# CSB5/XNA_Basecaller

Measured on NVIDIA B200. Metric: signal samples/sec basecalled (sup@v3.3 XNA), higher is better.
Workload: dtype fp16

## Files before the change

### include/xna_basecaller.h

```cpp
#ifndef XNA_BASECALLER_H
#define XNA_BASECALLER_H

#include <stdint.h>

#ifdef __cplusplus
extern "C" {
#endif

#define XB_ABI_VERSION 2

typedef struct xb_handle xb_handle;

enum xb_status {
    XB_OK = 0,
    XB_ERR_ARG = -1,
    XB_ERR_CUDA = -2,
    XB_ERR_STATE = -3,
    XB_ERR_UNSUPPORTED = -4,
    XB_ERR_NOMEM = -5
};

enum xb_flags {
    XB_FLAG_BF16 = 1,
    XB_FLAG_NO_ENCODER = 2,
// ... 73 lines not shown
int xb_encoder_fwd_train(xb_handle *h, const void *signal, int sig_dtype, int N, int L, float *scores, void *stream);
int xb_encoder_bwd(xb_handle *h, const void *signal, int sig_dtype, const float *scores, const float *dscores,
                   float *const *grads, int n_tensors, void *stream);

int xb_adamw_step(float *const *params, float *const *grads, float *const *exp_avg, float *const *exp_avg_sq,
                  const int64_t *numel, int n_tensors, float lr, float beta1, float beta2, float eps, float weight_decay,
                  float max_norm, int64_t step, float *grad_norm, float *scratch, void *stream);

int xb_stitch(xb_handle *h, const int8_t *rows, int T, const int32_t *chunk_first,
              const int32_t *chunk_count, const int32_t *read_len, int n_reads, int chunksize,
              int overlap, int stride, int reverse, int8_t *out, int out_stride, int32_t *out_len, void *stream);

int xb_gather_chunks(xb_handle *h, const void *signal, int sig_dtype, const int64_t *read_offset,
                     const int32_t *read_len, const int32_t *chunk_read, const int32_t *chunk_start, int n_chunks,
                     int L, float *out, void *stream);

int xb_preprocess_reads(xb_handle *h, const int16_t *raw, const int64_t *read_offset, const int32_t *read_len,
                        const double *scaling, const int32_t *offset, int n_reads, float *out, int32_t *out_len,
                        float *stats, void *stream);

int xb_compute_scores_host(xb_handle *h, const float *signal_host, int N, int L, int8_t *seq_host,
                           int32_t *lens_host, void *stream);

int xb_compute_scores_submit(xb_handle *h, int slot, const float *signal_host, int N, int L, int8_t *seq_host,
                             int32_t *lens_host, void *stream);
int xb_compute_scores_wait(xb_handle *h, int slot);

int64_t xb_launch_count(const xb_handle *h);

#define XB_NUM_STAGES 13
int xb_set_profiling(xb_handle *h, int on);
int xb_stage_times(xb_handle *h, float *ms, int *spans);

int xb_gemm_selftest(xb_handle *h, const void *A, const void *B, float *D, int M, int N, int K,
                     void *stream);

#ifdef __cplusplus
}
#endif
#endif
```

### xna_basecaller_b200/_lib.py

```python
import ctypes
import os

import torch

_HERE = os.path.dirname(os.path.abspath(__file__))
LIB_PATH = os.path.join(_HERE, 'libxna_b200.so')

XB_FLAG_BF16 = 1
XB_FLAG_NO_ENCODER = 2
XB_FLAG_TRAIN = 8
XB_SIG_F32, XB_SIG_F16, XB_SIG_I16 = 0, 1, 2
NUM_WEIGHTS = 28

SYMBOLS = (
    'xb_abi_version', 'xb_last_error', 'xb_create', 'xb_destroy', 'xb_load_weights', 'xb_load_conv_weights',
    'xb_load_lstm_weights', 'xb_load_head_weights', 'xb_conv_stem_fwd',
    'xb_lstm_fwd', 'xb_lstm_stack_fwd', 'xb_crf_head_fwd', 'xb_encoder_fwd', 'xb_crf_logz',
    'xb_crf_forward_scores', 'xb_crf_backward_scores', 'xb_crf_posteriors', 'xb_crf_viterbi', 'xb_crf_decode',
    'xb_ctc_crf_loss_fwd', 'xb_ctc_crf_loss_bwd', 'xb_stitch', 'xb_gather_chunks', 'xb_preprocess_reads', 'xb_compute_scores_host', 'xb_compute_scores_submit', 'xb_compute_scores_wait', 'xb_launch_count', 'xb_gemm_selftest',
    'xb_set_profiling', 'xb_stage_times', 'xb_crf_head_fwd_exp', 'xb_crf_decode_exp', 'xb_basecall_chunks',
    'xb_crf_logz_s', 'xb_crf_forward_scores_s', 'xb_crf_backward_scores_s', 'xb_crf_posteriors_max',
    'xb_encoder_fwd_train', 'xb_encoder_bwd', 'xb_adamw_step', 'xb_crf_beam_search',
)
STAGES = ('conv12_im2col', 'conv3_gemm', 'lstm_inproj_gemm', 'lstm_recurrence', 'crf_head_gemm', 'crf_alpha',
          'crf_backward', 'crf_viterbi', 'train_bptt', 'train_transpose', 'train_weight_grad_gemm', 'train_input_grad_gemm', 'train_head_conv_bwd')

_lib = None


def load():
    global _lib
    if _lib is not None:
        return _lib
    if not os.path.exists(LIB_PATH):
        raise RuntimeError(
            'xna_basecaller_b200: %s is missing -- build it with `python -m xna_basecaller_b200.build` '
            '(there is no CPU or PyTorch fallback for this path)' % LIB_PATH)
    lib = ctypes.CDLL(LIB_PATH)
    vp, ci, cf = ctypes.c_void_p, ctypes.c_int, ctypes.c_float
    lib.xb_abi_version.restype = ci
    lib.xb_last_error.restype = ctypes.c_char_p
    lib.xb_last_error.argtypes = [vp]
    lib.xb_create.argtypes = [ctypes.POINTER(vp), ci, ci, ci, ci, ci, ctypes.c_char_p, ci]
    lib.xb_destroy.argtypes = [vp]
    lib.xb_load_weights.argtypes = [vp, ctypes.POINTER(vp), ci, cf, cf, ci, vp]
    lib.xb_load_conv_weights.argtypes = [vp, vp, vp, vp, vp, vp, vp, vp]
    lib.xb_load_lstm_weights.argtypes = [vp, ci, vp, vp, vp, vp, vp]
    lib.xb_load_head_weights.argtypes = [vp, vp, vp, cf, cf, ci, vp]
    lib.xb_conv_stem_fwd.argtypes = [vp, vp, ci, ci, ci, vp, vp]
    lib.xb_lstm_fwd.argtypes = [vp, ci, vp, vp, ci, ci, ci, vp]
    lib.xb_lstm_stack_fwd.argtypes = [vp, vp, vp, ci, ci, vp]
    lib.xb_crf_head_fwd.argtypes = [vp, vp, vp, ci, ci, vp]
    lib.xb_encoder_fwd.argtypes = [vp, vp, ci, ci, ci, vp, vp]
    lib.xb_crf_logz.argtypes = [vp, vp, ci, ci, vp, vp]
    lib.xb_crf_forward_scores.argtypes = [vp, vp, ci, ci, vp, vp]
    lib.xb_crf_backward_scores.argtypes = [vp, vp, ci, ci, vp, vp]
    lib.xb_crf_posteriors.argtypes = [vp, vp, ci, ci, vp, vp]
    lib.xb_encoder_fwd_train.argtypes = [vp, vp, ci, ci, ci, vp, vp]
    lib.xb_encoder_bwd.argtypes = [vp, vp, ci, vp, vp, ctypes.POINTER(vp), ci, vp]
    lib.xb_adamw_step.argtypes = [ctypes.POINTER(vp), ctypes.POINTER(vp), ctypes.POINTER(vp), ctypes.POINTER(vp),
                                  ctypes.POINTER(ctypes.c_int64), ci, cf, cf, cf, cf, cf, cf, ctypes.c_int64, vp, vp, vp]
    lib.xb_crf_beam_search.argtypes = [vp, vp, ci, ci, ci, cf, vp, vp, vp, vp, vp]
    lib.xb_crf_logz_s.argtypes = [vp, vp, ci, ci, ci, vp, vp]
    lib.xb_crf_forward_scores_s.argtypes = [vp, vp, ci, ci, ci, vp, vp]
    lib.xb_crf_backward_scores_s.argtypes = [vp, vp, ci, ci, ci, vp, vp]
    lib.xb_crf_posteriors_max.argtypes = [vp, vp, ci, ci, vp, vp, vp]
    lib.xb_crf_viterbi.argtypes = [vp, vp, ci, ci, vp, vp]
    lib.xb_crf_decode.argtypes = [vp, vp, ci, ci, vp, vp, vp, vp, vp, vp]
    lib.xb_crf_decode_exp.argtypes = [vp, vp, ci, ci, vp, vp, vp, vp, vp, vp]
    lib.xb_crf_head_fwd_exp.argtypes = [vp, vp, vp, ci, ci, vp]
    lib.xb_basecall_chunks.argtypes = [vp, vp, ci, ci, ci, vp, vp, vp, vp]
    lib.xb_ctc_crf_loss_fwd.argtypes = [vp, vp, ci, ci, vp, ci, vp, ci, vp, vp]
    lib.xb_compute_scores_submit.argtypes = [vp, ci, vp, ci, ci, vp, vp, vp]
    lib.xb_compute_scores_wait.argtypes = [vp, ci]
    lib.xb_preprocess_reads.argtypes = [vp, vp, vp, vp, vp, vp, ci, vp, vp, vp, vp]
    lib.xb_ctc_crf_loss_bwd.argtypes = [vp, vp, ci, ci, vp, ci, vp, ci, vp, vp, vp, vp]
    lib.xb_stitch.argtypes = [vp, vp, ci, vp, vp, vp, ci, ci, ci, ci, ci, vp, ci, vp, vp]
    lib.xb_gather_chunks.argtypes = [vp, vp, ci, vp, vp, vp, vp, ci, ci, vp, vp]
    lib.xb_compute_scores_host.argtypes = [vp, vp, ci, ci, vp, vp, vp]
    lib.xb_launch_count.restype = ctypes.c_int64
    lib.xb_launch_count.argtypes = [vp]
    lib.xb_gemm_selftest.argtypes = [vp, vp, vp, vp, ci, ci, ci, vp]
    lib.xb_set_profiling.argtypes = [vp, ci]
    lib.xb_stage_times.argtypes = [vp, vp, vp]
    for name in SYMBOLS:
        if name not in ('xb_last_error', 'xb_launch_count'):
            getattr(lib, name).restype = ci
    _lib = lib
    return lib


def _ptr(t):
    return None if t is None else ctypes.c_void_p(t.data_ptr())


def _stream(device):
    return ctypes.c_void_p(torch.cuda.current_stream(device).cuda_stream)


class Handle:

    def __init__(self, alphabet, state_len=3, max_N=64, max_T=800, device=0, bf16=False, encoder=True, train=False):
        if not torch.cuda.is_available():
            raise RuntimeError('xna_basecaller_b200 needs a CUDA device (sm_100a); there is no CPU fallback')
        self.lib = load()
        self.alphabet = ''.join(alphabet)
        self.n_base = len(self.alphabet) - 1
        self.state_len = state_len
        self.C = self.n_base ** state_len
        self.NZ = self.n_base + 1
        self.max_N, self.max_T = max_N, max_T
        self.device = torch.device('cuda', device) if not isinstance(device, torch.device) else device
        self.bf16 = bf16
        self.dtype16 = torch.float16
        flags = (XB_FLAG_BF16 if bf16 else 0) | (0 if encoder else XB_FLAG_NO_ENCODER) | (XB_FLAG_TRAIN if train else 0)
        self.train = train
        h = ctypes.c_void_p()
        rc = self.lib.xb_create(ctypes.byref(h), self.device.index or 0, max_N, max_T, self.n_base, state_len,
                                self.alphabet.encode(), flags)
        if rc != 0:
            raise RuntimeError('xb_create failed (%d): %s' % (rc, self.lib.xb_last_error(None).decode()))
        self.h = h
        self._keep = None

    def close(self):
        if getattr(self, 'h', None):
            self.lib.xb_destroy(self.h)
            self.h = None

    def __del__(self):
        try:
            self.close()
        except Exception:
            pass

    def _check(self, rc, what):
        if rc != 0:
            raise RuntimeError('%s failed (%d): %s' % (what, rc, self.lib.xb_last_error(self.h).decode()))

    @property
    def launches(self):
        return int(self.lib.xb_launch_count(self.h))

    def set_profiling(self, on):
        self._check(self.lib.xb_set_profiling(self.h, int(on)), 'xb_set_profiling')

    def stage_times(self):
        ms = (ctypes.c_float * len(STAGES))()
        n = (ctypes.c_int * len(STAGES))()
        self._check(self.lib.xb_stage_times(self.h, ms, n), 'xb_stage_times')
        return {name: (float(ms[i]), int(n[i])) for i, name in enumerate(STAGES)}

    def load_weights(self, state_dict, scale=5.0, blank_score=2.0, expand_blanks=True):
        keys = []
        for i in range(3):
            keys += ['encoder.%d.conv.weight' % i, 'encoder.%d.conv.bias' % i]
        for i in range(4, 9):
            keys += ['encoder.%d.rnn.%s' % (i, k) for k in ('weight_ih_l0', 'weight_hh_l0', 'bias_ih_l0', 'bias_hh_l0')]
        keys += ['encoder.9.linear.weight', 'encoder.9.linear.bias']
        tensors = [state_dict[k].detach().to(self.device, torch.float32).contiguous() for k in keys]
        arr = (ctypes.c_void_p * NUM_WEIGHTS)(*[t.data_ptr() for t in tensors])
        rc = self.lib.xb_load_weights(self.h, arr, NUM_WEIGHTS, float(scale),
                                      float(blank_score if blank_score is not None else 0.0),
                                      int(bool(expand_blanks) and blank_score is not None), _stream(self.device))
        self._check(rc, 'xb_load_weights')
        torch.cuda.current_stream(self.device).synchronize()

    def _f32(self, t):
        return t.detach().to(self.device, torch.float32).contiguous()

    def load_conv_weights(self, w1, b1, w2, b2, w3, b3):
        ts = [self._f32(t) for t in (w1, b1, w2, b2, w3, b3)]
        self._check(self.lib.xb_load_conv_weights(self.h, *[_ptr(t) for t in ts], _stream(self.device)),
                    'xb_load_conv_weights')
        torch.cuda.current_stream(self.device).synchronize()

    def load_lstm_weights(self, layer, w_ih, w_hh, b_ih, b_hh):
        ts = [self._f32(t) for t in (w_ih, w_hh, b_ih, b_hh)]
        self._check(self.lib.xb_load_lstm_weights(self.h, int(layer), *[_ptr(t) for t in ts], _stream(self.device)),
# ... 271 lines not shown
```

### xna_basecaller_b200/csrc/lstm_persistent.cu

```cuda
#include <stdlib.h>

#include "xb_common.cuh"
#include "xb_ptx.cuh"
#include "xb_gemm.cuh"

using namespace xbptx;

#ifndef XB_LSTM_MUFU_TANH
#define XB_LSTM_MUFU_TANH 1
#endif

namespace {

constexpr int TILES = 24;
constexpr int KCH = XB_FEATURES / 64;
constexpr int HP = 3;
constexpr int KPB = KCH / HP;
constexpr int D_COL = 384;
constexpr int CTR_STRIDE = 32;
constexpr int MAX_CTRS = 64;

template <int SUB, int NS, int EW, int GB = 2> struct Cfg {
    static constexpr int NB = SUB * NS;
    static constexpr int H_BLOCK_BYTES = NS * 64 * 2;
    static constexpr int H_PART_BYTES = KPB * H_BLOCK_BYTES;
    static constexpr int H_BYTES = KCH * H_BLOCK_BYTES;
    static constexpr int G_BYTES = NS * 128 * 2;
    static constexpr int NBAR = HP + 1 + 4;
    static constexpr int EPI_WARP0 = ((SUB + 1 + 3) / 4) * 4;
    static constexpr int THREADS = (EPI_WARP0 + EW * SUB) * 32;
    static constexpr int NC = NS * 4 / EW;
    static constexpr int STAGE_BYTES = NC * 16;
    static constexpr int SMEM_BYTES = SUB * (H_BYTES + GB * G_BYTES) + (GB == 2 ? SUB * EW * STAGE_BYTES : 0) + 1024  + 1024 ;
    static_assert(D_COL + SUB * NS <= 512, "tensor memory columns");
    static_assert(NS % 16 == 0 && NS <= 48, "MMA N");
    static_assert((EW == 4 || EW == 8 || EW == 12) && NC % 16 == 0, "epilogue split");
    static_assert(SUB * NBAR * 8 + 16 <= 1024, "barrier block");
    static_assert(H_BLOCK_BYTES % 1024 == 0, "swizzle atom alignment");
};

struct PLParams {
    int T, N, reverse;
    int batch0, nbatch, G;
    const uint16_t *w_hh;
    uint16_t *y;
    int *counters;
    int one_release;
    int prefetch_y;
    long long *dbg;
    int tma_store;
    uint16_t *save;
};

#ifdef XB_EXPERIMENTS
#define DBG(sub_, ev) do { if (p.dbg && blockIdx.x == 0 && s >= 64 && s < 72) p.dbg[((s - 64) * 8 + (sub_)) * 16 + (ev)] = clock64(); } while (0)
#else
#define DBG(sub_, ev) do { } while (0)
#endif

__device__ __forceinline__ float tanh_approx(float x) {
    float y;
    asm("tanh.approx.f32 %0, %1;" : "=f"(y) : "f"(x));
    return y;
}
#if !XB_LSTM_MUFU_TANH
__device__ __forceinline__ float ex2f(float x) {
    float y;
    asm("ex2.approx.ftz.f32 %0, %1;" : "=f"(y) : "f"(x));
    return y;
}
__device__ __forceinline__ float rcpf(float x) {
    float y;
    asm("rcp.approx.ftz.f32 %0, %1;" : "=f"(y) : "f"(x));
    return y;
}
__device__ __forceinline__ float clampf(float x, float lim) { return fminf(fmaxf(x, -lim), lim); }
#endif

template <int XN> __device__ __forceinline__ void tmem_ld_16x256b(uint32_t taddr, uint32_t (&r)[4 * XN]);
template <> __device__ __forceinline__ void tmem_ld_16x256b<2>(uint32_t taddr, uint32_t (&r)[8]) {
    asm volatile("tcgen05.ld.sync.aligned.16x256b.x2.b32 {%0, %1, %2, %3, %4, %5, %6, %7}, [%8];"
                 : "=r"(r[0]), "=r"(r[1]), "=r"(r[2]), "=r"(r[3]), "=r"(r[4]), "=r"(r[5]), "=r"(r[6]), "=r"(r[7])
                 : "r"(taddr) : "memory");
}
template <> __device__ __forceinline__ void tmem_ld_16x256b<4>(uint32_t taddr, uint32_t (&r)[16]) {
    asm volatile("tcgen05.ld.sync.aligned.16x256b.x4.b32 {%0, %1, %2, %3, %4, %5, %6, %7, %8, %9, %10, %11, %12, %13, %14, %15}, [%16];"
                 : "=r"(r[0]), "=r"(r[1]), "=r"(r[2]), "=r"(r[3]), "=r"(r[4]), "=r"(r[5]), "=r"(r[6]), "=r"(r[7]), "=r"(r[8]),
                   "=r"(r[9]), "=r"(r[10]), "=r"(r[11]), "=r"(r[12]), "=r"(r[13]), "=r"(r[14]), "=r"(r[15])
                 : "r"(taddr) : "memory");
}
template <bool BF16, int SUB, int NS, int EW, int GB, bool SAVE = false>
__global__ void __launch_bounds__(Cfg<SUB, NS, EW, GB>::THREADS, 1)
lstm_persistent_kernel(const __grid_constant__ CUtensorMap tmY, const __grid_constant__ CUtensorMap tmG,
                       const __grid_constant__ CUtensorMap tmS, const PLParams p) {
    using X = xb16<BF16>;
    using C = Cfg<SUB, NS, EW, GB>;
    extern __shared__ uint8_t smem_raw[];
    uint8_t *smem = reinterpret_cast<uint8_t *>((reinterpret_cast<uintptr_t>(smem_raw) + 1023) & ~uintptr_t(1023));
    uint8_t *hbuf = smem;
    uint8_t *gbuf = smem + SUB * C::H_BYTES;
    uint8_t *stage = gbuf + SUB * GB * C::G_BYTES;
    uint64_t *bars = reinterpret_cast<uint64_t *>(stage + (GB == 2 ? SUB * EW * C::STAGE_BYTES : 0));
    uint32_t *tmem_holder = reinterpret_cast<uint32_t *>(bars + SUB * C::NBAR);
    auto h_full = [&](int sub, int part) { return bars + sub * C::NBAR + part; };
    auto d_full = [&](int sub) { return bars + sub * C::NBAR + HP; };
    auto g_full = [&](int sub, int q) { return bars + sub * C::NBAR + HP + 1 + q; };
    auto g_empty = [&](int sub, int q) { return bars + sub * C::NBAR + HP + 3 + q; };

    const int warp = __shfl_sync(0xffffffffu, (int)(threadIdx.x >> 5), 0), lane = threadIdx.x & 31;
    const int g = blockIdx.x / TILES, j = blockIdx.x % TILES;
    const int T = p.T, N = p.N;
    const int units = (p.nbatch + NS - 1) / NS;
    const int b0 = p.batch0 + NS * (int)(((long long)g * units) / p.G);
    const int b1 = min(p.batch0 + p.nbatch, p.batch0 + NS * (int)(((long long)(g + 1) * units) / p.G));
    const int count = b1 - b0;
    auto sub_row0 = [&](int sub) { return b0 + sub * NS; };
    auto sub_cnt = [&](int sub) { return max(0, min(NS, count - sub * NS)); };

    if (warp == 0 && lane == 0) {
        prefetch_tmap(&tmY);
        prefetch_tmap(&tmG);
        for (int sub = 0; sub < SUB; sub++) {
            for (int part = 0; part < HP; part++) mbar_init(h_full(sub, part), 1);
            mbar_init(d_full(sub), 1);
            for (int q = 0; q < 2; q++) {
                mbar_init(g_full(sub, q), 1);
                mbar_init(g_empty(sub, q), EW);
            }
        }
        fence_barrier_init();
    }
    if (warp == SUB) {
        tmem_alloc(tmem_holder, 512);
        tmem_relinquish();
    }
    tc_fence_before();
    __syncthreads();
    tc_fence_after();
    const uint32_t tmem_base = *tmem_holder;

    if (warp >= C::EPI_WARP0 && warp < C::EPI_WARP0 + 4) {
        const int q = warp & 3, r = q * 32 + lane;
        const uint4 *src = reinterpret_cast<const uint4 *>(p.w_hh + ((size_t)j * 128 + r) * XB_FEATURES);
        const uint32_t taddr = tmem_base + ((uint32_t)(q * 32) << 16);
#pragma unroll 1
        for (int c0 = 0; c0 < XB_FEATURES / 2; c0 += 32) {
            uint32_t v[32];
#pragma unroll
            for (int i = 0; i < 8; i++) {
                uint4 t4 = __ldg(src + c0 / 4 + i);
                v[4 * i] = t4.x; v[4 * i + 1] = t4.y; v[4 * i + 2] = t4.z; v[4 * i + 3] = t4.w;
            }
            tmem_st_32x32b_x32(taddr + c0, v);
        }
        tmem_st_wait();
    }
    tc_fence_before();
    __syncthreads();
    tc_fence_after();

    if (warp < SUB) {
        if (elect_one()) {
            const int sub = warp;
            const int row0 = sub_row0(sub);
            const int cnt_sub = sub_cnt(sub);
            const int *ctr = p.counters + (g * SUB + sub) * CTR_STRIDE;
            uint8_t *hb = hbuf + sub * C::H_BYTES;
            constexpr uint32_t idesc = umma_idesc_f16(BF16 ? 1u : 0u, 128, NS);
            const uint64_t bdesc0 = umma_desc_sw128(smem_u32(hb));
            const uint32_t dcol = tmem_base + D_COL + sub * NS;
            if (cnt_sub > 0) {
                mbar_expect_tx(g_full(sub, 0), C::G_BYTES);
                tma_load_2d(gbuf + (sub * GB) * C::G_BYTES, &tmG, g_full(sub, 0), j * 128, (p.reverse ? T - 1 : 0) * N + row0);
            }
            for (int s = 0; s < (cnt_sub > 0 ? T : 0); s++) {
                const int t = p.reverse ? T - 1 - s : s;
                if (GB == 2 && s + 1 < T) {
                    const int sn = s + 1, q = sn & 1, u = sn >> 1;
                    const int tn = p.reverse ? T - 1 - sn : sn;
                    if (u >= 1) mbar_wait(g_empty(sub, q), (u - 1) & 1);
                    mbar_expect_tx(g_full(sub, q), C::G_BYTES);
                    tma_load_2d(gbuf + (sub * 2 + q) * C::G_BYTES, &tmG, g_full(sub, q), j * 128, tn * N + row0);
                }
                if (p.prefetch_y && s + p.prefetch_y < T) {
                    const int t2 = p.reverse ? T - 1 - (s + p.prefetch_y) : s + p.prefetch_y;
                    for (int r = j; r < cnt_sub; r += TILES)
                        prefetch_l2_bulk(p.y + ((size_t)t2 * N + row0 + r) * XB_FEATURES, XB_FEATURES * 2);
                }
                if (s > 0) {
                    const int tp = p.reverse ? t + 1 : t - 1;
                    const int need = TILES * EW * s;
                    DBG(sub, 0);
                    while (ld_relaxed_gpu(ctr) < need) {
                    }
                    (void)ld_acquire_gpu(ctr);
                    DBG(sub, 1);
                    fence_proxy_async_global();
#pragma unroll
                    for (int part = 0; part < HP; part++) {
                        mbar_expect_tx(h_full(sub, part), C::H_PART_BYTES);
                        tma_load_3d(hb + part * C::H_PART_BYTES, &tmY, h_full(sub, part), 0, tp * N + row0, part * KPB);
                    }
                    DBG(sub, 2);
#pragma unroll
                    for (int part = 0; part < HP; part++) {
                        mbar_wait(h_full(sub, part), (s - 1) & 1);
                        tc_fence_after();
                        if (part == 0) DBG(sub, 8);
                        if (part == 0) DBG(sub, 3);
#pragma unroll
                        for (int kk = 0; kk < KPB * 4; kk++) {
                            const int kc = kk >> 2, k = kk & 3;
                            mma_f16_ts(dcol, tmem_base + part * (KPB * 32) + kk * 8,
                                       bdesc0 + (uint64_t)((part * C::H_PART_BYTES + kc * C::H_BLOCK_BYTES + k * 32) >> 4), idesc,
                                       (part | kk) != 0);
                        }
                    }
                    mma_commit(d_full(sub));
                    DBG(sub, 4);
                }
                if (GB == 1 && s + 1 < T) {
                    const int tn = p.reverse ? T - 2 - s : s + 1;
                    mbar_wait(g_empty(sub, 0), s & 1);
                    mbar_expect_tx(g_full(sub, 0), C::G_BYTES);
                    tma_load_2d(gbuf + sub * C::G_BYTES, &tmG, g_full(sub, 0), j * 128, tn * N + row0);
                }
            }
        }
    } else if (warp >= C::EPI_WARP0) {
        constexpr int NC = C::NC, CELLS = NC / 4;
        const int ew = (warp - C::EPI_WARP0) % EW, sub = (warp - C::EPI_WARP0) / EW, q = warp & 3;
        const int col0 = (ew >> 2) * NC;
        const int gt = lane & 3, ul = lane >> 2;
        const int unit = q * 8 + ul;
        const int row0 = sub_row0(sub);
        const int cnt = sub_cnt(sub);
#ifdef XB_EXPERIMENTS
        const bool tma_store = !SAVE && GB == 2 && cnt == NS && p.tma_store;
#else
        constexpr bool tma_store = false;
#endif
        const uint32_t taddr = tmem_base + ((uint32_t)(q * 32) << 16) + D_COL + sub * NS + col0;
        int *ctr = p.counters + (g * SUB + sub) * CTR_STRIDE;
        float cst[CELLS];
#pragma unroll
        for (int i = 0; i < CELLS; i++) cst[i] = 0.0f;

        for (int s = 0; s < (cnt > 0 ? T : 0); s++) {
            const int t = p.reverse ? T - 1 - s : s;
            const uint16_t *Gs = reinterpret_cast<const uint16_t *>(gbuf + (sub * GB + (GB == 2 ? (s & 1) : 0)) * C::G_BYTES);
            mbar_wait(g_full(sub, GB == 2 ? (s & 1) : 0), GB == 2 ? ((s >> 1) & 1) : (s & 1));
// ... 113 lines not shown
                if (ew == 0 && lane == 0) {
                    red_release_gpu_add(ctr, EW);
                    DBG(sub, 13);
                }
                if (lane == 0) mbar_arrive(g_empty(sub, GB == 2 ? (s & 1) : 0));
            } else {
                __syncwarp();
                if (lane == 0) {
                    red_release_gpu_add(ctr, 1);
                    mbar_arrive(g_empty(sub, GB == 2 ? (s & 1) : 0));
                    if (ew == 0) DBG(sub, 13);
                }
            }
            if (SAVE) {
                static_assert(!SAVE || GB == 2, "the saved-state stores reuse the staging rows after the gate buffer has been released");
#pragma unroll
                for (int qn = 0; qn < 5; qn++) {
                    __syncwarp();
#pragma unroll
                    for (int i = 0; i < CELLS; i++) {
                        const __half hv = __float2half_rn(sv[SAVE ? qn : 0][i]);
                        sts_u16(st_s + 2u * ((8 * (i >> 1) + 2 * gt + (i & 1)) * ST_PITCH + ul), *reinterpret_cast<const uint16_t *>(&hv));
                    }
                    __syncwarp();
                    if (lane < NC && col0 + lane < cnt)
                        *reinterpret_cast<uint4 *>(p.save + (((size_t)t * N + row0 + col0 + lane) * 5 + qn) * XB_FEATURES + j * 32 + q * 8) =
                            lds_v4(st_s + 2u * (lane * ST_PITCH));
                }
            }
        }
    }
    tc_fence_before();
    __syncthreads();
    if (warp == SUB) {
        tc_fence_after();
        tmem_dealloc(tmem_base, 512);
    }
}

template <bool BF16, int SUB, int NS, int EW, int GB = 2, bool SAVE = false>
int launch_cfg(xb_handle *h, int layer, void *y_tnc, int T, int N, int reverse, cudaStream_t s, void *save = nullptr) {
    using C = Cfg<SUB, NS, EW, GB>;
    CUtensorMap tmY, tmG, tmS;
    if (int rc = xb_make_tmap_hview(h, &tmY, y_tnc, (uint64_t)T * N, NS, KPB)) return rc;
    if (int rc = xb_make_tmap_2d_box(h, &tmS, y_tnc, (uint64_t)T * N, XB_FEATURES, XB_FEATURES, 32, NS, 0)) return rc;
    if (int rc = xb_make_tmap_2d_box(h, &tmG, h->gates, (uint64_t)T * N, XB_GATES, XB_GATES, 128, NS, 0)) return rc;
    const int max_groups = h->num_sms / TILES;
    if (max_groups < 1)
        return xb_fail(h, XB_ERR_UNSUPPORTED, "the persistent LSTM needs %d co-resident CTAs, the device has %d SMs", TILES, h->num_sms);
    const int block_cap = max_groups * C::NB;
    auto fn = lstm_persistent_kernel<BF16, SUB, NS, EW, GB, SAVE>;
    static bool configured[64] = {};
    if (!configured[h->device & 63]) {
        XB_CUDA(h, cudaFuncSetAttribute(fn, cudaFuncAttributeMaxDynamicSharedMemorySize, C::SMEM_BYTES));
        configured[h->device & 63] = true;
    }
    for (int batch0 = 0; batch0 < N; batch0 += block_cap) {
        PLParams p;
        p.T = T; p.N = N; p.reverse = reverse;
        p.batch0 = batch0;
        p.nbatch = (N - batch0 < block_cap) ? N - batch0 : block_cap;
        p.G = (p.nbatch + C::NB - 1) / C::NB;
        p.w_hh = reinterpret_cast<const uint16_t *>(h->lstm[layer].w_hh);
        p.y = reinterpret_cast<uint16_t *>(y_tnc);
        p.counters = h->lstm_counters;
        p.one_release = 1;
        p.prefetch_y = 4;
        p.dbg = nullptr;
        p.save = reinterpret_cast<uint16_t *>(save);
        p.tma_store = 0;
#ifdef XB_EXPERIMENTS
        if (getenv("XB_TMAS")) p.tma_store = atoi(getenv("XB_TMAS"));
#endif
#ifdef XB_EXPERIMENTS
        if (getenv("XB_LSTM_WARP_RELEASE")) p.one_release = 0;
        if (getenv("XB_LSTM_PREFETCH_Y")) p.prefetch_y = atoi(getenv("XB_LSTM_PREFETCH_Y"));
        if (getenv("XB_LSTM_DEBUG")) p.dbg = reinterpret_cast<long long *>(h->lstm_counters + MAX_CTRS * CTR_STRIDE);
#endif
        XB_CUDA(h, cudaMemsetAsync(h->lstm_counters, 0, MAX_CTRS * CTR_STRIDE * sizeof(int), s));
        void *args[] = {(void *)&tmY, (void *)&tmG, (void *)&tmS, (void *)&p};
        XB_CUDA(h, cudaLaunchCooperativeKernel((const void *)fn, dim3(p.G * TILES), dim3(C::THREADS), args, C::SMEM_BYTES, s));
        h->launches++;
    }
    return XB_OK;
}

}

#ifdef XB_EXPERIMENTS
extern "C" int xb_debug_lstm_timeline(xb_handle *h, long long *out_host) {
    if (!h || !h->lstm_counters) return XB_ERR_STATE;
    XB_CUDA(h, cudaDeviceSynchronize());
    XB_CUDA(h, cudaMemcpy(out_host, h->lstm_counters + MAX_CTRS * CTR_STRIDE, 8 * 8 * 16 * sizeof(long long), cudaMemcpyDeviceToHost));
    return XB_OK;
}
#endif

int xb_lstm_recurrence_persistent(xb_handle *h, int layer, void *y_tnc, int T, int N, int reverse, cudaStream_t s, void *save) {
    if (!h->lstm_counters) {
        void *q = nullptr;
        XB_CUDA(h, cudaMalloc(&q, MAX_CTRS * CTR_STRIDE * sizeof(int) + 8 * 8 * 16 * sizeof(long long)));
        h->lstm_counters = reinterpret_cast<int *>(q);
    }
#ifdef XB_EXPERIMENTS
    static const int variant = getenv("XB_LSTM_VARIANT") ? atoi(getenv("XB_LSTM_VARIANT")) : 0;
    if (variant == 1)
        return launch_cfg<false, 3, 32, 4>(h, layer, y_tnc, T, N, reverse, s);
    if (variant == 4)
        return launch_cfg<false, 4, 32, 4, 1>(h, layer, y_tnc, T, N, reverse, s);
    if (variant == 3)
        return launch_cfg<false, 2, 48, 12>(h, layer, y_tnc, T, N, reverse, s);
    if (variant == 2)
        return launch_cfg<false, 6, 16, 4>(h, layer, y_tnc, T, N, reverse, s);
#endif
    if (save) return launch_cfg<false, 3, 32, 8, 2, true>(h, layer, y_tnc, T, N, reverse, s, save);
    return launch_cfg<false, 3, 32, 8>(h, layer, y_tnc, T, N, reverse, s);
}
```

### xna_basecaller_b200/csrc/xb_common.cuh

```cuda
#pragma once

#include <cuda_runtime.h>
#include <cuda_fp16.h>
#include <cuda_bf16.h>
#include <cuda.h>
#include <stdint.h>
#include <stdio.h>
#include <string>
#include <vector>

#include "../../include/xna_basecaller.h"

#define XB_FEATURES 768
#define XB_GATES (4 * XB_FEATURES)
#define XB_STRIDE 5
#define XB_WINLEN 19
#define XB_C2_CH 16
#define XB_C2_HALO 9
#define XB_CONV3_K 320

struct xb_lstm_weights {
    void *w_ih = nullptr;
    void *w_hh = nullptr;
    float *bias = nullptr;
// ... 25 lines not shown
    float *conv1_w = nullptr, *conv1_b = nullptr, *conv2_w = nullptr, *conv2_b = nullptr;
    void *conv3_w = nullptr;
    float *conv3_b = nullptr;
    xb_lstm_weights lstm[5];
    void *head_w = nullptr;
    float *head_b = nullptr;
    int head_rows = 0, head_rows_padded = 0;
    float scale = 5.0f, blank_score = 2.0f;
    int expand_blanks = 1;

    void *c2 = nullptr;
    void *act0 = nullptr, *act1 = nullptr;
    void *gates = nullptr;
    float *cstate = nullptr;
    void *hzero = nullptr;
    float *scores = nullptr;
    void *signal_dev = nullptr;
    int8_t *seq_dev = nullptr;
    int32_t *lens_dev = nullptr;
    void *signal_dev2 = nullptr;
    int8_t *seq_dev2 = nullptr;
    int32_t *lens_dev2 = nullptr;
    cudaStream_t h2d_stream = nullptr, d2h_stream = nullptr;
    cudaEvent_t ev_h2d[2] = {nullptr, nullptr}, ev_enc[2] = {nullptr, nullptr}, ev_dec[2] = {nullptr, nullptr},
                ev_done[2] = {nullptr, nullptr};
    bool slot_used[2] = {false, false};

    float *alpha = nullptr;
    float *bmax = nullptr;
    float *lp = nullptr;
    float *logz = nullptr;
    float *ctc_ws = nullptr;
    int *lstm_counters = nullptr;

    void *head_wT = nullptr;
    void *conv3_wT = nullptr;
    struct xb_train_ws *train = nullptr;

    void *encode_tiled = nullptr;
};

extern thread_local std::string xb_global_err;

struct xb_stage_timer {
    xb_handle *h; cudaStream_t s; int idx = -1;
    xb_stage_timer(xb_handle *h_, int stage, cudaStream_t s_) : h(h_), s(s_) {
        if (!h->profiling) return;
        auto get = [&]() { cudaEvent_t e; if (!h->event_pool.empty()) { e = h->event_pool.back(); h->event_pool.pop_back(); }
                           else cudaEventCreate(&e); return e; };
        xb_prof_span sp{stage, get(), get()};
        cudaEventRecord(sp.a, s);
        h->spans.push_back(sp);
        idx = (int)h->spans.size() - 1;
    }
    ~xb_stage_timer() { if (idx >= 0) cudaEventRecord(h->spans[idx].b, s); }
};

int xb_fail(xb_handle *h, int code, const char *fmt, ...);

#define XB_CUDA(h, call)                                                                         \
    do {                                                                                         \
        cudaError_t e_ = (call);                                                                 \
        if (e_ != cudaSuccess)                                                                   \
            return xb_fail((h), XB_ERR_CUDA, "%s failed: %s (%s:%d)", #call, cudaGetErrorString(e_), \
                           __FILE__, __LINE__);                                                  \
    } while (0)
// ... 51 lines not shown
```

### xna_basecaller_b200/csrc/xb_ptx.cuh

```cuda
#pragma once
#include <cuda.h>
#include <stdint.h>

namespace xbptx {

__device__ __forceinline__ uint32_t smem_u32(const void *p) { return (uint32_t)__cvta_generic_to_shared(p); }

__device__ __forceinline__ bool elect_one() {
    uint32_t pred;
    asm volatile(
        "{\n\t.reg .pred P;\n\t.reg .b32 R;\n\t"
        "elect.sync R|P, 0xffffffff;\n\t"
        "selp.b32 %0, 1, 0, P;\n\t}"
        : "=r"(pred));
    return pred != 0;
}

__device__ __forceinline__ void mbar_init(uint64_t *bar, uint32_t count) {
    asm volatile("mbarrier.init.shared::cta.b64 [%0], %1;" ::"r"(smem_u32(bar)), "r"(count));
}
__device__ __forceinline__ void fence_barrier_init() { asm volatile("fence.mbarrier_init.release.cluster;" ::: "memory"); }
__device__ __forceinline__ void fence_proxy_async() { asm volatile("fence.proxy.async.shared::cta;" ::: "memory"); }
__device__ __forceinline__ void fence_proxy_async_all() { asm volatile("fence.proxy.async;" ::: "memory"); }
__device__ __forceinline__ void fence_proxy_async_global() { asm volatile("fence.proxy.async.global;" ::: "memory"); }
// ... 76 lines not shown
}
__device__ __forceinline__ void tma_load_2d(void *dst, const CUtensorMap *m, uint64_t *bar, int c0, int c1) {
    asm volatile(
        "cp.async.bulk.tensor.2d.shared::cluster.global.mbarrier::complete_tx::bytes [%0], [%1, {%3, %4}], [%2];"
        ::"r"(smem_u32(dst)), "l"(m), "r"(smem_u32(bar)), "r"(c0), "r"(c1)
        : "memory");
}
__device__ __forceinline__ void tma_load_3d(void *dst, const CUtensorMap *m, uint64_t *bar, int c0, int c1, int c2) {
    asm volatile(
        "cp.async.bulk.tensor.3d.shared::cluster.global.mbarrier::complete_tx::bytes [%0], [%1, {%3, %4, %5}], [%2];"
        ::"r"(smem_u32(dst)), "l"(m), "r"(smem_u32(bar)), "r"(c0), "r"(c1), "r"(c2)
        : "memory");
}

__device__ __forceinline__ void tma_store_2d(const CUtensorMap *m, uint32_t src_smem, int c0, int c1) {
    asm volatile("cp.async.bulk.tensor.2d.global.shared::cta.bulk_group [%0, {%2, %3}], [%1];"
                 ::"l"(m), "r"(src_smem), "r"(c0), "r"(c1) : "memory");
}
__device__ __forceinline__ void tma_load_4d(void *dst, const CUtensorMap *m, uint64_t *bar, int c0, int c1, int c2, int c3) {
    asm volatile(
        "cp.async.bulk.tensor.4d.shared::cluster.global.mbarrier::complete_tx::bytes [%0], [%1, {%3, %4, %5, %6}], [%2];"
        ::"r"(smem_u32(dst)), "l"(m), "r"(smem_u32(bar)), "r"(c0), "r"(c1), "r"(c2), "r"(c3)
        : "memory");
}
__device__ __forceinline__ void tma_store_4d(const CUtensorMap *m, uint32_t src_smem, int c0, int c1, int c2, int c3) {
    asm volatile("cp.async.bulk.tensor.4d.global.shared::cta.bulk_group [%0, {%2, %3, %4, %5}], [%1];"
                 ::"l"(m), "r"(src_smem), "r"(c0), "r"(c1), "r"(c2), "r"(c3) : "memory");
}
__device__ __forceinline__ void griddep_launch_dependents() { asm volatile("griddepcontrol.launch_dependents;" ::: "memory"); }
__device__ __forceinline__ void griddep_wait() { asm volatile("griddepcontrol.wait;" ::: "memory"); }
__device__ __forceinline__ void bulk_commit_group() { asm volatile("cp.async.bulk.commit_group;" ::: "memory"); }
__device__ __forceinline__ void bulk_wait_group0() { asm volatile("cp.async.bulk.wait_group 0;" ::: "memory"); }

__device__ __forceinline__ void tmem_alloc(uint32_t *holder_smem, uint32_t ncols) {
    asm volatile("tcgen05.alloc.cta_group::1.sync.aligned.shared::cta.b32 [%0], %1;" ::"r"(smem_u32(holder_smem)), "r"(ncols)
                 : "memory");
}
__device__ __forceinline__ void tmem_relinquish() {
    asm volatile("tcgen05.relinquish_alloc_permit.cta_group::1.sync.aligned;" ::: "memory");
}
__device__ __forceinline__ void tmem_dealloc(uint32_t taddr, uint32_t ncols) {
    asm volatile("tcgen05.dealloc.cta_group::1.sync.aligned.b32 %0, %1;" ::"r"(taddr), "r"(ncols) : "memory");
}
__device__ __forceinline__ void tc_fence_before() { asm volatile("tcgen05.fence::before_thread_sync;" ::: "memory"); }
__device__ __forceinline__ void tc_fence_after() { asm volatile("tcgen05.fence::after_thread_sync;" ::: "memory"); }

__device__ __forceinline__ void mma_f16_ss(uint32_t d_tmem, uint64_t adesc, uint64_t bdesc, uint32_t idesc, uint32_t accumulate) {
    asm volatile(
        "{\n\t.reg .pred p;\n\t"
        "setp.ne.b32 p, %4, 0;\n\t"
        "tcgen05.mma.cta_group::1.kind::f16 [%0], %1, %2, %3, p;\n\t}"
        ::"r"(d_tmem), "l"(adesc), "l"(bdesc), "r"(idesc), "r"(accumulate)
        : "memory");
}
__device__ __forceinline__ void mma_f16_ts(uint32_t d_tmem, uint32_t a_tmem, uint64_t bdesc, uint32_t idesc, uint32_t accumulate) {
    asm volatile(
        "{\n\t.reg .pred p;\n\t"
        "setp.ne.b32 p, %4, 0;\n\t"
        "tcgen05.mma.cta_group::1.kind::f16 [%0], [%1], %2, %3, p;\n\t}"
        ::"r"(d_tmem), "r"(a_tmem), "l"(bdesc), "r"(idesc), "r"(accumulate)
        : "memory");
}
__device__ __forceinline__ void tmem_cp_128x256b(uint32_t taddr, uint64_t sdesc) {
    asm volatile("tcgen05.cp.cta_group::1.128x256b [%0], %1;" ::"r"(taddr), "l"(sdesc) : "memory");
}
__device__ __forceinline__ void mma_commit(uint64_t *bar) {
    asm volatile("tcgen05.commit.cta_group::1.mbarrier::arrive::one.shared::cluster.b64 [%0];" ::"r"(smem_u32(bar)) : "memory");
}

__device__ __forceinline__ void tmem_ld_32x32b_x32(uint32_t taddr, uint32_t (&r)[32]) {
    asm volatile(
        "tcgen05.ld.sync.aligned.32x32b.x32.b32 "
        "{%0, %1, %2, %3, %4, %5, %6, %7, %8, %9, %10, %11, %12, %13, %14, %15, "
        "%16, %17, %18, %19, %20, %21, %22, %23, %24, %25, %26, %27, %28, %29, %30, %31}, [%32];"
        : "=r"(r[0]), "=r"(r[1]), "=r"(r[2]), "=r"(r[3]), "=r"(r[4]), "=r"(r[5]), "=r"(r[6]), "=r"(r[7]), "=r"(r[8]),
          "=r"(r[9]), "=r"(r[10]), "=r"(r[11]), "=r"(r[12]), "=r"(r[13]), "=r"(r[14]), "=r"(r[15]), "=r"(r[16]),
          "=r"(r[17]), "=r"(r[18]), "=r"(r[19]), "=r"(r[20]), "=r"(r[21]), "=r"(r[22]), "=r"(r[23]), "=r"(r[24]),
          "=r"(r[25]), "=r"(r[26]), "=r"(r[27]), "=r"(r[28]), "=r"(r[29]), "=r"(r[30]), "=r"(r[31])
        : "r"(taddr)
        : "memory");
}
__device__ __forceinline__ void tmem_ld_32x32b_x8(uint32_t taddr, uint32_t (&r)[8]) {
    asm volatile("tcgen05.ld.sync.aligned.32x32b.x8.b32 {%0, %1, %2, %3, %4, %5, %6, %7}, [%8];"
                 : "=r"(r[0]), "=r"(r[1]), "=r"(r[2]), "=r"(r[3]), "=r"(r[4]), "=r"(r[5]), "=r"(r[6]), "=r"(r[7])
                 : "r"(taddr)
                 : "memory");
}
__device__ __forceinline__ void tmem_ld_32x32b_x16(uint32_t taddr, uint32_t (&r)[16]) {
    asm volatile(
        "tcgen05.ld.sync.aligned.32x32b.x16.b32 "
        "{%0, %1, %2, %3, %4, %5, %6, %7, %8, %9, %10, %11, %12, %13, %14, %15}, [%16];"
        : "=r"(r[0]), "=r"(r[1]), "=r"(r[2]), "=r"(r[3]), "=r"(r[4]), "=r"(r[5]), "=r"(r[6]), "=r"(r[7]), "=r"(r[8]),
          "=r"(r[9]), "=r"(r[10]), "=r"(r[11]), "=r"(r[12]), "=r"(r[13]), "=r"(r[14]), "=r"(r[15])
        : "r"(taddr)
// ... 30 lines not shown
```

Baseline: 83.64 million.

## Run persistent LSTM recurrence as 2-CTA cluster pairs with cta_group::2 UMMA

Adds a PAIR variant of the persistent LSTM kernel that launches 2-CTA clusters. It allocates tensor memory with cta_group::2 and loads each CTA's half of the hidden state with a paired TMA that signals the leader's barrier. Only rank 0 then issues M=256 MMAs and a multicast commit. This halves the per-CTA hidden-state buffer and should reduce per-step MMA issue overhead in the recurrent loop. It is enabled by default when occupancy checks show the clusters can be co-resident. The cost is cluster synchronisation and the risk of mixing cta_group::1 and cta_group::2 tcgen05 operations.

```diff
diff --git a/include/xna_basecaller.h b/include/xna_basecaller.h
--- a/include/xna_basecaller.h
+++ b/include/xna_basecaller.h
@@ -129,6 +129,8 @@
 int xb_set_profiling(xb_handle *h, int on);
 int xb_stage_times(xb_handle *h, float *ms, int *spans);
 
+int xb_set_lstm_pairs(xb_handle *h, int on);
+
 int xb_gemm_selftest(xb_handle *h, const void *A, const void *B, float *D, int M, int N, int K,
                      void *stream);
 
diff --git a/xna_basecaller_b200/_lib.py b/xna_basecaller_b200/_lib.py
--- a/xna_basecaller_b200/_lib.py
+++ b/xna_basecaller_b200/_lib.py
@@ -20,7 +20,7 @@
     'xb_ctc_crf_loss_fwd', 'xb_ctc_crf_loss_bwd', 'xb_stitch', 'xb_gather_chunks', 'xb_preprocess_reads', 'xb_compute_scores_host', 'xb_compute_scores_submit', 'xb_compute_scores_wait', 'xb_launch_count', 'xb_gemm_selftest',
     'xb_set_profiling', 'xb_stage_times', 'xb_crf_head_fwd_exp', 'xb_crf_decode_exp', 'xb_basecall_chunks',
     'xb_crf_logz_s', 'xb_crf_forward_scores_s', 'xb_crf_backward_scores_s', 'xb_crf_posteriors_max',
-    'xb_encoder_fwd_train', 'xb_encoder_bwd', 'xb_adamw_step', 'xb_crf_beam_search',
+    'xb_encoder_fwd_train', 'xb_encoder_bwd', 'xb_adamw_step', 'xb_crf_beam_search', 'xb_set_lstm_pairs',
 )
 STAGES = ('conv12_im2col', 'conv3_gemm', 'lstm_inproj_gemm', 'lstm_recurrence', 'crf_head_gemm', 'crf_alpha',
           'crf_backward', 'crf_viterbi', 'train_bptt', 'train_transpose', 'train_weight_grad_gemm', 'train_input_grad_gemm', 'train_head_conv_bwd')
@@ -83,6 +83,7 @@
     lib.xb_gemm_selftest.argtypes = [vp, vp, vp, vp, ci, ci, ci, vp]
     lib.xb_set_profiling.argtypes = [vp, ci]
     lib.xb_stage_times.argtypes = [vp, vp, vp]
+    lib.xb_set_lstm_pairs.argtypes = [vp, ci]
     for name in SYMBOLS:
         if name not in ('xb_last_error', 'xb_launch_count'):
             getattr(lib, name).restype = ci
@@ -145,6 +146,9 @@
     def set_profiling(self, on):
         self._check(self.lib.xb_set_profiling(self.h, int(on)), 'xb_set_profiling')
 
+    def set_lstm_pairs(self, on):
+        self._check(self.lib.xb_set_lstm_pairs(self.h, int(on)), 'xb_set_lstm_pairs')
+
     def stage_times(self):
         ms = (ctypes.c_float * len(STAGES))()
         n = (ctypes.c_int * len(STAGES))()
diff --git a/xna_basecaller_b200/csrc/lstm_persistent.cu b/xna_basecaller_b200/csrc/lstm_persistent.cu
--- a/xna_basecaller_b200/csrc/lstm_persistent.cu
+++ b/xna_basecaller_b200/csrc/lstm_persistent.cu
@@ -20,9 +20,10 @@
 constexpr int CTR_STRIDE = 32;
 constexpr int MAX_CTRS = 64;
 
-template <int SUB, int NS, int EW, int GB = 2> struct Cfg {
+template <int SUB, int NS, int EW, int GB = 2, bool PAIR = false> struct Cfg {
     static constexpr int NB = SUB * NS;
-    static constexpr int H_BLOCK_BYTES = NS * 64 * 2;
+    static constexpr int HN = PAIR ? NS / 2 : NS;
+    static constexpr int H_BLOCK_BYTES = HN * 64 * 2;
     static constexpr int H_PART_BYTES = KPB * H_BLOCK_BYTES;
     static constexpr int H_BYTES = KCH * H_BLOCK_BYTES;
     static constexpr int G_BYTES = NS * 128 * 2;
@@ -89,12 +90,13 @@
                    "=r"(r[9]), "=r"(r[10]), "=r"(r[11]), "=r"(r[12]), "=r"(r[13]), "=r"(r[14]), "=r"(r[15])
                  : "r"(taddr) : "memory");
 }
-template <bool BF16, int SUB, int NS, int EW, int GB, bool SAVE = false>
-__global__ void __launch_bounds__(Cfg<SUB, NS, EW, GB>::THREADS, 1)
+template <bool BF16, int SUB, int NS, int EW, int GB, bool SAVE = false, bool PAIR = false>
+__global__ void __launch_bounds__(Cfg<SUB, NS, EW, GB, PAIR>::THREADS, 1)
 lstm_persistent_kernel(const __grid_constant__ CUtensorMap tmY, const __grid_constant__ CUtensorMap tmG,
                        const __grid_constant__ CUtensorMap tmS, const PLParams p) {
     using X = xb16<BF16>;
-    using C = Cfg<SUB, NS, EW, GB>;
+    using C = Cfg<SUB, NS, EW, GB, PAIR>;
+    constexpr int CG = PAIR ? 2 : 1;
     extern __shared__ uint8_t smem_raw[];
     uint8_t *smem = reinterpret_cast<uint8_t *>((reinterpret_cast<uintptr_t>(smem_raw) + 1023) & ~uintptr_t(1023));
     uint8_t *hbuf = smem;
@@ -131,13 +133,15 @@
         fence_barrier_init();
     }
     if (warp == SUB) {
-        tmem_alloc(tmem_holder, 512);
-        tmem_relinquish();
+        tmem_alloc<CG>(tmem_holder, 512);
+        tmem_relinquish<CG>();
     }
     tc_fence_before();
     __syncthreads();
+    if (PAIR) cluster_sync();
     tc_fence_after();
     const uint32_t tmem_base = *tmem_holder;
+    const uint32_t rank = PAIR ? cluster_ctarank() : 0;
 
     if (warp >= C::EPI_WARP0 && warp < C::EPI_WARP0 + 4) {
         const int q = warp & 3, r = q * 32 + lane;
@@ -166,7 +170,7 @@
             const int cnt_sub = sub_cnt(sub);
             const int *ctr = p.counters + (g * SUB + sub) * CTR_STRIDE;
             uint8_t *hb = hbuf + sub * C::H_BYTES;
-            constexpr uint32_t idesc = umma_idesc_f16(BF16 ? 1u : 0u, 128, NS);
+            constexpr uint32_t idesc = umma_idesc_f16(BF16 ? 1u : 0u, PAIR ? 256 : 128, NS);
             const uint64_t bdesc0 = umma_desc_sw128(smem_u32(hb));
             const uint32_t dcol = tmem_base + D_COL + sub * NS;
             if (cnt_sub > 0) {
@@ -198,25 +202,35 @@
                     fence_proxy_async_global();
 #pragma unroll
                     for (int part = 0; part < HP; part++) {
-                        mbar_expect_tx(h_full(sub, part), C::H_PART_BYTES);
-                        tma_load_3d(hb + part * C::H_PART_BYTES, &tmY, h_full(sub, part), 0, tp * N + row0, part * KPB);
+                        if (PAIR) {
+                            if (rank == 0) mbar_expect_tx(h_full(sub, part), 2 * C::H_PART_BYTES);
+                            tma_load_3d_pair(hb + part * C::H_PART_BYTES, &tmY, mapa_shared(smem_u32(h_full(sub, part)), 0), 0,
+                                             tp * N + row0 + (int)rank * C::HN, part * KPB);
+                        } else {
+                            mbar_expect_tx(h_full(sub, part), C::H_PART_BYTES);
+                            tma_load_3d(hb + part * C::H_PART_BYTES, &tmY, h_full(sub, part), 0, tp * N + row0, part * KPB);
+                        }
                     }
                     DBG(sub, 2);
-#pragma unroll
-                    for (int part = 0; part < HP; part++) {
-                        mbar_wait(h_full(sub, part), (s - 1) & 1);
-                        tc_fence_after();
-                        if (part == 0) DBG(sub, 8);
-                        if (part == 0) DBG(sub, 3);
-#pragma unroll
-                        for (int kk = 0; kk < KPB * 4; kk++) {
-                            const int kc = kk >> 2, k = kk & 3;
-                            mma_f16_ts(dcol, tmem_base + part * (KPB * 32) + kk * 8,
-                                       bdesc0 + (uint64_t)((part * C::H_PART_BYTES + kc * C::H_BLOCK_BYTES + k * 32) >> 4), idesc,
-                                       (part | kk) != 0);
+                    if (rank == 0) {
+#pragma unroll
+                        for (int part = 0; part < HP; part++) {
+                            mbar_wait(h_full(sub, part), (s - 1) & 1);
+                            tc_fence_after();
+                            if (part == 0) DBG(sub, 8);
+                            if (part == 0) DBG(sub, 3);
+#pragma unroll
+                            for (int kk = 0; kk < KPB * 4; kk++) {
+                                const int kc = kk >> 2, k = kk & 3;
+                                const uint32_t a = tmem_base + part * (KPB * 32) + kk * 8;
+                                const uint64_t b = bdesc0 + (uint64_t)((part * C::H_PART_BYTES + kc * C::H_BLOCK_BYTES + k * 32) >> 4);
+                                if (PAIR) mma_f16_ts_pair(dcol, a, b, idesc, (part | kk) != 0);
+                                else mma_f16_ts(dcol, a, b, idesc, (part | kk) != 0);
+                            }
                         }
+                        if (PAIR) mma_commit_pair(d_full(sub));
+                        else mma_commit(d_full(sub));
                     }
-                    mma_commit(d_full(sub));
                     DBG(sub, 4);
                 }
                 if (GB == 1 && s + 1 < T) {
@@ -396,29 +410,51 @@
     }
     tc_fence_before();
     __syncthreads();
+    if (PAIR) cluster_sync();
     if (warp == SUB) {
         tc_fence_after();
-        tmem_dealloc(tmem_base, 512);
-    }
-}
-
-template <bool BF16, int SUB, int NS, int EW, int GB = 2, bool SAVE = false>
+        tmem_dealloc<CG>(tmem_base, 512);
+    }
+}
+
+template <bool BF16, int SUB, int NS, int EW, int GB, bool SAVE, bool PAIR> int resident_groups(xb_handle *h) {
+    using C = Cfg<SUB, NS, EW, GB, PAIR>;
+    auto fn = lstm_persistent_kernel<BF16, SUB, NS, EW, GB, SAVE, PAIR>;
+    static int groups[64];
+    static bool configured[64] = {};
+    if (configured[h->device & 63]) return groups[h->device & 63];
+    XB_CUDA(h, cudaFuncSetAttribute(fn, cudaFuncAttributeMaxDynamicSharedMemorySize, C::SMEM_BYTES));
+    int g = h->num_sms / TILES;
+    if (PAIR) {
+        cudaLaunchAttribute attr[1];
+        attr[0].id = cudaLaunchAttributeClusterDimension;
+        attr[0].val.clusterDim.x = 2; attr[0].val.clusterDim.y = 1; attr[0].val.clusterDim.z = 1;
+        cudaLaunchConfig_t cfg = {};
+        cfg.gridDim = dim3(g * TILES); cfg.blockDim = dim3(C::THREADS); cfg.dynamicSmemBytes = C::SMEM_BYTES;
+        cfg.attrs = attr; cfg.numAttrs = 1;
+        int clusters = 0;
+        XB_CUDA(h, cudaOccupancyMaxActiveClusters(&clusters, (const void *)fn, &cfg));
+        if (2 * clusters / TILES < g) g = 0;
+    }
+    groups[h->device & 63] = g;
+    configured[h->device & 63] = true;
+    return g;
+}
+
+template <bool BF16, int SUB, int NS, int EW, int GB = 2, bool SAVE = false, bool PAIR = false>
 int launch_cfg(xb_handle *h, int layer, void *y_tnc, int T, int N, int reverse, cudaStream_t s, void *save = nullptr) {
-    using C = Cfg<SUB, NS, EW, GB>;
+    using C = Cfg<SUB, NS, EW, GB, PAIR>;
     CUtensorMap tmY, tmG, tmS;
-    if (int rc = xb_make_tmap_hview(h, &tmY, y_tnc, (uint64_t)T * N, NS, KPB)) return rc;
+    if (int rc = xb_make_tmap_hview(h, &tmY, y_tnc, (uint64_t)T * N, C::HN, KPB)) return rc;
     if (int rc = xb_make_tmap_2d_box(h, &tmS, y_tnc, (uint64_t)T * N, XB_FEATURES, XB_FEATURES, 32, NS, 0)) return rc;
     if (int rc = xb_make_tmap_2d_box(h, &tmG, h->gates, (uint64_t)T * N, XB_GATES, XB_GATES, 128, NS, 0)) return rc;
-    const int max_groups = h->num_sms / TILES;
+    const int max_groups = resident_groups<BF16, SUB, NS, EW, GB, SAVE, PAIR>(h);
+    if (max_groups < 0) return max_groups;
     if (max_groups < 1)
-        return xb_fail(h, XB_ERR_UNSUPPORTED, "the persistent LSTM needs %d co-resident CTAs, the device has %d SMs", TILES, h->num_sms);
+        return xb_fail(h, XB_ERR_UNSUPPORTED, "the persistent LSTM%s needs %d co-resident CTAs, the device has %d SMs",
+                       PAIR ? " (CTA pairs)" : "", TILES, h->num_sms);
     const int block_cap = max_groups * C::NB;
-    auto fn = lstm_persistent_kernel<BF16, SUB, NS, EW, GB, SAVE>;
-    static bool configured[64] = {};
-    if (!configured[h->device & 63]) {
-        XB_CUDA(h, cudaFuncSetAttribute(fn, cudaFuncAttributeMaxDynamicSharedMemorySize, C::SMEM_BYTES));
-        configured[h->device & 63] = true;
-    }
+    auto fn = lstm_persistent_kernel<BF16, SUB, NS, EW, GB, SAVE, PAIR>;
     for (int batch0 = 0; batch0 < N; batch0 += block_cap) {
         PLParams p;
         p.T = T; p.N = N; p.reverse = reverse;
@@ -443,7 +479,15 @@
 #endif
         XB_CUDA(h, cudaMemsetAsync(h->lstm_counters, 0, MAX_CTRS * CTR_STRIDE * sizeof(int), s));
         void *args[] = {(void *)&tmY, (void *)&tmG, (void *)&tmS, (void *)&p};
-        XB_CUDA(h, cudaLaunchCooperativeKernel((const void *)fn, dim3(p.G * TILES), dim3(C::THREADS), args, C::SMEM_BYTES, s));
+        cudaLaunchAttribute attr[2];
+        attr[0].id = cudaLaunchAttributeCooperative;
+        attr[0].val.cooperative = 1;
+        attr[1].id = cudaLaunchAttributeClusterDimension;
+        attr[1].val.clusterDim.x = 2; attr[1].val.clusterDim.y = 1; attr[1].val.clusterDim.z = 1;
+        cudaLaunchConfig_t cfg = {};
+        cfg.gridDim = dim3(p.G * TILES); cfg.blockDim = dim3(C::THREADS); cfg.dynamicSmemBytes = C::SMEM_BYTES; cfg.stream = s;
+        cfg.attrs = attr; cfg.numAttrs = PAIR ? 2 : 1;
+        XB_CUDA(h, cudaLaunchKernelExC(&cfg, (const void *)fn, args));
         h->launches++;
     }
     return XB_OK;
@@ -477,6 +521,29 @@
     if (variant == 2)
         return launch_cfg<false, 6, 16, 4>(h, layer, y_tnc, T, N, reverse, s);
 #endif
-    if (save) return launch_cfg<false, 3, 32, 8, 2, true>(h, layer, y_tnc, T, N, reverse, s, save);
+    if (h->lstm_pairs < 0) {
+        const int rc = xb_set_lstm_pairs(h, 1);
+        if (rc != XB_OK && rc != XB_ERR_UNSUPPORTED) return rc;
+        if (rc != XB_OK) h->lstm_pairs = 0;
+    }
+    if (save) {
+        if (h->lstm_pairs) return launch_cfg<false, 3, 32, 8, 2, true, true>(h, layer, y_tnc, T, N, reverse, s, save);
+        return launch_cfg<false, 3, 32, 8, 2, true>(h, layer, y_tnc, T, N, reverse, s, save);
+    }
+    if (h->lstm_pairs) return launch_cfg<false, 3, 32, 8, 2, false, true>(h, layer, y_tnc, T, N, reverse, s);
     return launch_cfg<false, 3, 32, 8>(h, layer, y_tnc, T, N, reverse, s);
 }
+
+extern "C" int xb_set_lstm_pairs(xb_handle *h, int on) {
+    if (!h) return xb_fail(nullptr, XB_ERR_ARG, "NULL handle");
+    if (on) {
+        int g = resident_groups<false, 3, 32, 8, 2, false, true>(h);
+        if (g > 0) g = resident_groups<false, 3, 32, 8, 2, true, true>(h);
+        if (g < 0) return g;
+        if (g == 0)
+            return xb_fail(h, XB_ERR_UNSUPPORTED, "xb_set_lstm_pairs: this device cannot co-schedule the %d CTA pairs of %d groups",
+                           h->num_sms / TILES * TILES / 2, h->num_sms / TILES);
+    }
+    h->lstm_pairs = on ? 1 : 0;
+    return XB_OK;
+}
diff --git a/xna_basecaller_b200/csrc/xb_common.cuh b/xna_basecaller_b200/csrc/xb_common.cuh
--- a/xna_basecaller_b200/csrc/xb_common.cuh
+++ b/xna_basecaller_b200/csrc/xb_common.cuh
@@ -81,6 +81,7 @@
     float *logz = nullptr;
     float *ctc_ws = nullptr;
     int *lstm_counters = nullptr;
+    int lstm_pairs = -1;
 
     void *head_wT = nullptr;
     void *conv3_wT = nullptr;
diff --git a/xna_basecaller_b200/csrc/xb_ptx.cuh b/xna_basecaller_b200/csrc/xb_ptx.cuh
--- a/xna_basecaller_b200/csrc/xb_ptx.cuh
+++ b/xna_basecaller_b200/csrc/xb_ptx.cuh
@@ -132,15 +132,41 @@
 __device__ __forceinline__ void bulk_commit_group() { asm volatile("cp.async.bulk.commit_group;" ::: "memory"); }
 __device__ __forceinline__ void bulk_wait_group0() { asm volatile("cp.async.bulk.wait_group 0;" ::: "memory"); }
 
-__device__ __forceinline__ void tmem_alloc(uint32_t *holder_smem, uint32_t ncols) {
-    asm volatile("tcgen05.alloc.cta_group::1.sync.aligned.shared::cta.b32 [%0], %1;" ::"r"(smem_u32(holder_smem)), "r"(ncols)
-                 : "memory");
-}
-__device__ __forceinline__ void tmem_relinquish() {
-    asm volatile("tcgen05.relinquish_alloc_permit.cta_group::1.sync.aligned;" ::: "memory");
-}
-__device__ __forceinline__ void tmem_dealloc(uint32_t taddr, uint32_t ncols) {
-    asm volatile("tcgen05.dealloc.cta_group::1.sync.aligned.b32 %0, %1;" ::"r"(taddr), "r"(ncols) : "memory");
+__device__ __forceinline__ uint32_t cluster_ctarank() {
+    uint32_t r;
+    asm volatile("mov.u32 %0, %%cluster_ctarank;" : "=r"(r));
+    return r;
+}
+__device__ __forceinline__ uint32_t mapa_shared(uint32_t saddr, uint32_t rank) {
+    uint32_t r;
+    asm volatile("mapa.shared::cluster.u32 %0, %1, %2;" : "=r"(r) : "r"(saddr), "r"(rank));
+    return r;
+}
+__device__ __forceinline__ void cluster_sync() {
+    asm volatile("barrier.cluster.arrive.release.aligned;\n\tbarrier.cluster.wait.acquire.aligned;" ::: "memory");
+}
+__device__ __forceinline__ void tma_load_3d_pair(void *dst, const CUtensorMap *m, uint32_t bar_cluster, int c0, int c1, int c2) {
+    asm volatile(
+        "cp.async.bulk.tensor.3d.cta_group::2.shared::cluster.global.mbarrier::complete_tx::bytes [%0], [%1, {%3, %4, %5}], [%2];"
+        ::"r"(smem_u32(dst)), "l"(m), "r"(bar_cluster), "r"(c0), "r"(c1), "r"(c2)
+        : "memory");
+}
+
+template <int CG = 1> __device__ __forceinline__ void tmem_alloc(uint32_t *holder_smem, uint32_t ncols) {
+    if constexpr (CG == 1)
+        asm volatile("tcgen05.alloc.cta_group::1.sync.aligned.shared::cta.b32 [%0], %1;" ::"r"(smem_u32(holder_smem)), "r"(ncols)
+                     : "memory");
+    else
+        asm volatile("tcgen05.alloc.cta_group::2.sync.aligned.shared::cta.b32 [%0], %1;" ::"r"(smem_u32(holder_smem)), "r"(ncols)
+                     : "memory");
+}
+template <int CG = 1> __device__ __forceinline__ void tmem_relinquish() {
+    if constexpr (CG == 1) asm volatile("tcgen05.relinquish_alloc_permit.cta_group::1.sync.aligned;" ::: "memory");
+    else asm volatile("tcgen05.relinquish_alloc_permit.cta_group::2.sync.aligned;" ::: "memory");
+}
+template <int CG = 1> __device__ __forceinline__ void tmem_dealloc(uint32_t taddr, uint32_t ncols) {
+    if constexpr (CG == 1) asm volatile("tcgen05.dealloc.cta_group::1.sync.aligned.b32 %0, %1;" ::"r"(taddr), "r"(ncols) : "memory");
+    else asm volatile("tcgen05.dealloc.cta_group::2.sync.aligned.b32 %0, %1;" ::"r"(taddr), "r"(ncols) : "memory");
 }
 __device__ __forceinline__ void tc_fence_before() { asm volatile("tcgen05.fence::before_thread_sync;" ::: "memory"); }
 __device__ __forceinline__ void tc_fence_after() { asm volatile("tcgen05.fence::after_thread_sync;" ::: "memory"); }
@@ -160,6 +186,18 @@
         "tcgen05.mma.cta_group::1.kind::f16 [%0], [%1], %2, %3, p;\n\t}"
         ::"r"(d_tmem), "r"(a_tmem), "l"(bdesc), "r"(idesc), "r"(accumulate)
         : "memory");
+}
+__device__ __forceinline__ void mma_f16_ts_pair(uint32_t d_tmem, uint32_t a_tmem, uint64_t bdesc, uint32_t idesc, uint32_t accumulate) {
+    asm volatile(
+        "{\n\t.reg .pred p;\n\t"
+        "setp.ne.b32 p, %4, 0;\n\t"
+        "tcgen05.mma.cta_group::2.kind::f16 [%0], [%1], %2, %3, p;\n\t}"
+        ::"r"(d_tmem), "r"(a_tmem), "l"(bdesc), "r"(idesc), "r"(accumulate)
+        : "memory");
+}
+__device__ __forceinline__ void mma_commit_pair(uint64_t *bar) {
+    asm volatile("tcgen05.commit.cta_group::2.mbarrier::arrive::one.shared::cluster.multicast::cluster.b64 [%0], %1;"
+                 ::"r"(smem_u32(bar)), "h"((uint16_t)0x3) : "memory");
 }
 __device__ __forceinline__ void tmem_cp_128x256b(uint32_t taddr, uint64_t sdesc) {
     asm volatile("tcgen05.cp.cta_group::1.128x256b [%0], %1;" ::"r"(taddr), "l"(sdesc) : "memory");
```

New measurement: 84.39 million (median of 6 runs). Within noise of the previous version (+0.9%).
